# ai4sre/RCAEval

Hardware: AMD Instinct MI355X
Metric: Fisher-z CI tests/sec + PC skeleton wall-time (2000 vars), 1/2/4/8 MI355X (higher is better)
Workload: dtype f64

## Files before the change

include/pcgpu.h:

```cpp
#ifndef PCGPU_H
#define PCGPU_H

#include <stdint.h>

#ifdef __cplusplus
extern "C" {
#endif

#define PCG_OK 0
#define PCG_ERR_INVALID -1
#define PCG_ERR_OOM -2
#define PCG_ERR_HIP -3
#define PCG_ERR_SINGULAR -4
#define PCG_ERR_DOMAIN -5
#define PCG_ERR_RCCL -6
#define PCG_ERR_OVERFLOW -7
#define PCG_ERR_PEER -8

#define PCG_FLAG_FULL_P 0x1
#define PCG_FLAG_RECORD 0x2
#define PCG_FLAG_EXACT_ALL 0x4

#define PCG_MAX_LEVELS 32
#define PCG_MAX_DEPTH 12
// ... 12 lines not shown
    double level_ms[PCG_MAX_LEVELS];
    double kernel_ms[PCG_MAX_LEVELS];
    int32_t levels;
    int32_t error;
    int64_t screened[PCG_MAX_LEVELS];
    int32_t driver;
    int32_t driver_pad;
} pcg_stats;

#define PCG_DRIVER_LEVELS 0
#define PCG_DRIVER_SMALL 1
#define PCG_DRIVER_SMALL_RERUN 2

typedef struct {
    int32_t a, b;
    int32_t d;
    int32_t s[PCG_MAX_DEPTH];
    double p;
} pcg_record;

#define PCG_ABI_VERSION 4
int pcg_abi_info(int64_t *stats_bytes, int64_t *record_bytes, int32_t *version);

int pcg_create(int device, pcg_handle **out);
int pcg_destroy(pcg_handle *h);
const char *pcg_last_error(pcg_handle *h);
int pcg_set_stream(pcg_handle *h, void *hip_stream);
int pcg_set_capacity(pcg_handle *h, int64_t record_capacity, int64_t deferred_capacity);
int pcg_set_record_sample(pcg_handle *h, int64_t modulus, int64_t residue);

#define PCG_TUNE_SMALL 0
#define PCG_TUNE_SMALL_QCAP 1
#define PCG_TUNE_LDS_DEEP 2
#define PCG_TUNE_LDS_SPILL_MIN 3
#define PCG_TUNE_WAVE_LO 4
#define PCG_TUNE_SCREEN_MASK 5
#define PCG_TUNE_NODE_BLOCKS 6
#define PCG_TUNE_EXPORT_INLINE 7
#define PCG_TUNE_NB 8
#define PCG_TUNE_NBW 9
#define PCG_TUNE_HOST_TRACE 10
#define PCG_TUNE_K1_I8 11
#define PCG_TUNE_K1_CRT 12
#define PCG_TUNE_K1_CRT_MINN 13
#define PCG_TUNE_K1_CRT_BITS 14
#define PCG_TUNE_K1_CRT_KS 15
#define PCG_TUNE_K1_I8_KS 16
#define PCG_TUNE_K1_SUPER_ORDER 17
#define PCG_TUNE_L1Z 18
#define PCG_TUNE_K1_CRT_MIX 19
#define PCG_K1_CRT_MIX_FORCED (1ll << 30)
#define PCG_K1_CRT_MIX_FORCE(tA, ksA, ksB) \
    (PCG_K1_CRT_MIX_FORCED | ((int64_t)(tA) << 10) | ((int64_t)(ksA) << 5) | (int64_t)(ksB))
#define PCG_TUNE_COUNT 20
int pcg_set_tuning(pcg_handle *h, int key, int64_t value);
int pcg_get_tuning(pcg_handle *h, int key, int64_t *value);

int pcg_corr(pcg_handle *h, const double *X, int64_t N, int64_t n, int64_t ldx,
             double *C, int64_t ldc);

int pcg_corr_shard_bytes(pcg_handle *h, int64_t n, int64_t N, int world, int64_t *bytes_per_rank);
int pcg_k1_plan_signature(pcg_handle *h, int64_t n, int64_t N, int64_t *signature);
int pcg_k1_crt_plan(pcg_handle *h, int64_t n, int64_t N, int64_t *plan);
int pcg_corr_shard_rows(int64_t n, int world, int64_t *rows_per_rank);
int pcg_corr_shard(pcg_handle *h, const double *X, int64_t N, int64_t n, int64_t ldx, int rank,
                   int world, double *packed);
int pcg_corr_shard_finish(pcg_handle *h, const double *gathered, int64_t N, int64_t n, int world,
                          double *C, int64_t ldc);

int pcg_skeleton(pcg_handle *h, const double *C, int64_t n, int64_t ldc, int64_t N,
                 double alpha, int max_depth, int flags, int8_t *removed_level,
                 pcg_stats *stats);

int pcg_pc_skeleton(pcg_handle *h, const double *X, int64_t N, int64_t n, int64_t ldx, double *C,
                    int64_t ldc, double alpha, int max_depth, int flags, int8_t *removed_level,
                    pcg_stats *stats);

int pcg_degrees(pcg_handle *h, int32_t *deg_host, int64_t capacity);

int pcg_sepset_count(pcg_handle *h, int64_t *count, int32_t *words_per_row);
int pcg_sepset_export(pcg_handle *h, int32_t *xy_host ,
                      uint64_t *bits_host , int64_t count);
int pcg_sepset_export_device(pcg_handle *h, int32_t *xy_dev, uint64_t *bits_dev, int64_t count);
int pcg_set_sepset_buffers(pcg_handle *h, int32_t *xy_dev, uint64_t *bits_dev, int64_t capacity);
int pcg_sepset_target(pcg_handle *h, int32_t *in_caller, int64_t *capacity_needed);

int pcg_record_count(pcg_handle *h, int64_t *count, int64_t *near_alpha_count);
int pcg_record_export(pcg_handle *h, pcg_record *rec_host, int64_t count,
                      pcg_record *near_host, int64_t near_count);

typedef struct {
    const double *X;
    int64_t N, n, ldx;
    double *C;
    int64_t ldc;
    int8_t *removed_level;
    int32_t *sep_xy;
    uint64_t *sep_bits;
} pcg_case;
typedef struct {
    int32_t rc;
    int32_t rc_pad;
    int64_t sep_rows;
    int64_t near_alpha_count;
    pcg_stats stats;
    int32_t deg[PCG_MAX_LEVELS][64];
} pcg_case_result;
// ... 121 lines not shown
```

rcaeval_amd/_lib.py:

```python
from __future__ import annotations

import ctypes
import os

_HERE = os.path.dirname(os.path.abspath(__file__))
LIB_PATH = os.environ.get("PCG_LIB_PATH") or os.path.join(_HERE, "libpcgpu.so")

PCG_OK = 0
PCG_ERR_INVALID = -1
PCG_ERR_OOM = -2
PCG_ERR_HIP = -3
PCG_ERR_SINGULAR = -4
PCG_ERR_DOMAIN = -5
PCG_ERR_RCCL = -6
PCG_ERR_OVERFLOW = -7
PCG_ERR_PEER = -8

PCG_FLAG_FULL_P = 0x1
PCG_FLAG_RECORD = 0x2
PCG_FLAG_EXACT_ALL = 0x4

PCG_MAX_LEVELS = 32
PCG_ABI_VERSION = 4
PCG_RM_STATUS = 64
PCG_MAX_DEPTH = 12
PCG_MAX_LEVEL_DEPTH = 30

PCG_DRIVER_LEVELS = 0
PCG_DRIVER_SMALL = 1
PCG_DRIVER_SMALL_RERUN = 2
DRIVER_NAMES = {PCG_DRIVER_LEVELS: "levels", PCG_DRIVER_SMALL: "small", PCG_DRIVER_SMALL_RERUN: "small_rerun"}

TUNE_KEYS = {
    "SMALL": 0, "SMALL_QCAP": 1, "LDS_DEEP": 2, "LDS_SPILL_MIN": 3, "WAVE_LO": 4, "SCREEN_MASK": 5,
    "NODE_BLOCKS": 6, "EXPORT_INLINE": 7, "NB": 8, "NBW": 9, "HOST_TRACE": 10, "K1_I8": 11, "K1_CRT": 12,
    "K1_CRT_MINN": 13, "K1_CRT_BITS": 14, "K1_CRT_KS": 15, "K1_I8_KS": 16, "K1_SUPER_ORDER": 17,
    "L1Z": 18, "K1_CRT_MIX": 19,
}


def k1_crt_mix_force(tA: int, ksA: int, ksB: int) -> int:
    return (1 << 30) | (int(tA) << 10) | (int(ksA) << 5) | int(ksB)

I64 = ctypes.c_int64
I32 = ctypes.c_int32
P = ctypes.c_void_p
D = ctypes.c_double


class PcgStats(ctypes.Structure):
    _fields_ = [
        ("tests", I64 * PCG_MAX_LEVELS),
        ("calls", I64 * PCG_MAX_LEVELS),
        ("indep", I64 * PCG_MAX_LEVELS),
        ("exact", I64 * PCG_MAX_LEVELS),
        ("near_alpha", I64 * PCG_MAX_LEVELS),
        ("edges_after", I64 * PCG_MAX_LEVELS),
        ("max_degree", I32 * PCG_MAX_LEVELS),
        ("level_ms", D * PCG_MAX_LEVELS),
        ("kernel_ms", D * PCG_MAX_LEVELS),
        ("levels", I32),
        ("error", I32),
        ("screened", I64 * PCG_MAX_LEVELS),
        ("driver", I32),
        ("driver_pad", I32),
    ]

    def as_dict(self) -> dict:
        L = self.levels
        return {
            "levels": L,
            "error": self.error,
            "tests": list(self.tests[:L]),
            "calls": list(self.calls[:L]),
            "indep": list(self.indep[:L]),
            "exact": list(self.exact[:L]),
            "near_alpha": list(self.near_alpha[:L]),
            "edges_after": list(self.edges_after[:L]),
            "max_degree": list(self.max_degree[:L]),
            "level_ms": list(self.level_ms[:L]),
            "kernel_ms": list(self.kernel_ms[:L]),
            "screened": list(self.screened[:L]),
            "driver": DRIVER_NAMES.get(self.driver, str(self.driver)),
        }


class PcgRecord(ctypes.Structure):
    _fields_ = [("a", I32), ("b", I32), ("d", I32), ("s", I32 * PCG_MAX_DEPTH), ("p", D)]


# ... 176 lines not shown
```

rcaeval_amd/csrc/api.hip:

```cpp
#include <hip/hip_runtime.h>

#include <algorithm>
#include <cerrno>
#include <cstdlib>
#include <cstring>

#include "handle.h"

int pcg_fail(pcg_handle *h, int code, const char *fmt, ...) {
    if (h) {
        char buf[1024];
        va_list ap;
        va_start(ap, fmt);
        vsnprintf(buf, sizeof(buf), fmt, ap);
        va_end(ap);
        h->err = buf;
    }
    return code;
}

bool pcg_ensure(pcg_handle *h, DevBuf &b, size_t bytes) {
    if (bytes == 0) bytes = 16;
    if (b.bytes >= bytes) return true;
    if (b.p) {
// ... 25 lines not shown
    ++h->alloc_events;
    if (hipHostMalloc(&b.p, bytes, hipHostMallocMapped) != hipSuccess) {
        b.p = nullptr;
        return false;
    }
    if (hipHostGetDevicePointer(&b.dp, b.p, 0) != hipSuccess) {
        hipHostFree(b.p);
        b.p = b.dp = nullptr;
        return false;
    }
    b.bytes = bytes;
    return true;
}

extern "C" int pcg_abi_info(int64_t *stats_bytes, int64_t *record_bytes, int32_t *version) {
    if (stats_bytes) *stats_bytes = (int64_t)sizeof(pcg_stats);
    if (record_bytes) *record_bytes = (int64_t)sizeof(pcg_record);
    if (version) *version = PCG_ABI_VERSION;
    return PCG_OK;
}

extern "C" int pcg_batch_abi_info(int64_t *case_bytes, int64_t *result_bytes) {
    if (case_bytes) *case_bytes = (int64_t)sizeof(pcg_case);
    if (result_bytes) *result_bytes = (int64_t)sizeof(pcg_case_result);
    return PCG_OK;
}

namespace {
struct TuneSpec {
    const char *env;
    int64_t dflt, lo, hi;
};
const TuneSpec kTune[PCG_TUNE_COUNT] = {
    {"PCG_SMALL", 1, 0, 1},
    {"PCG_SMALL_QCAP", 1024, 1, 1024},
    {"PCG_LDS_DEEP", 20, 12, 20},
    {"PCG_LDS_SPILL_MIN", 10000000, 0, INT64_MAX},
    {"PCG_WAVE_LO", 0, 0, PCG_MAX_LEVEL_DEPTH + 1},
    {"PCG_SCREEN_MASK", -1, -1, 0x1c},
    {"PCG_NODE_BLOCKS", 0x18, 0, 0x1c},
    {"PCG_EXPORT_INLINE", 16384, 0, INT64_MAX},
    {"PCG_NB", 0, 0, 1 << 24},
    {"PCG_NBW", 512, 1, 1 << 24},
    {"PCG_HOST_TRACE", 0, 0, 1},
    {"PCG_K1_I8", 1, 0, 1},
    {"PCG_K1_CRT", 1, 0, 1},
    {"PCG_K1_CRT_MINN", 256, 1, 1 << 24},
    {"PCG_K1_CRT_BITS", 53, 32, 63},
    {"PCG_K1_CRT_KS", 0, 0, 16},
    {"PCG_K1_I8_KS", 0, 0, 256},
    {"PCG_K1_SUPER_ORDER", 1, 0, 1},
    {"PCG_L1Z", 1, 0, 1},
    {"PCG_K1_CRT_MIX", 1, 0, INT32_MAX},
};
}

void pcg_tuning_defaults(int64_t *tune) {
    for (int k = 0; k < PCG_TUNE_COUNT; ++k) {
        int64_t v = kTune[k].dflt;
        if (const char *e = getenv(kTune[k].env)) {
            char *end = nullptr;
            errno = 0;
            const long long p = strtoll(e, &end, 0);
            if (end == e || *end != '\0' || errno == ERANGE || p < kTune[k].lo || p > kTune[k].hi)
                fprintf(stderr, "pcgpu: ignoring %s=%s (not an integer in [%lld, %lld]); using %lld\n", kTune[k].env, e,
                        (long long)kTune[k].lo, (long long)kTune[k].hi, (long long)kTune[k].dflt);
            else
                v = p;
        }
        tune[k] = v;
    }
}

extern "C" int pcg_set_tuning(pcg_handle *h, int key, int64_t value) {
    if (!h || key < 0 || key >= PCG_TUNE_COUNT || value < kTune[key].lo || value > kTune[key].hi)
        return pcg_fail(h, PCG_ERR_INVALID, "pcg_set_tuning: key %d value %lld", key, (long long)value);
    h->tune[key] = value;
    return PCG_OK;
}

extern "C" int pcg_get_tuning(pcg_handle *h, int key, int64_t *value) {
    if (!h || !value || key < 0 || key >= PCG_TUNE_COUNT)
        return pcg_fail(h, PCG_ERR_INVALID, "pcg_get_tuning: key %d", key);
    *value = h->tune[key];
    return PCG_OK;
}

extern "C" int pcg_create(int device, pcg_handle **out) {
    if (!out) return PCG_ERR_INVALID;
    *out = nullptr;
    int ndev = 0;
    if (hipGetDeviceCount(&ndev) != hipSuccess || ndev <= 0) return PCG_ERR_HIP;
    if (device < 0 || device >= ndev) return PCG_ERR_INVALID;
    if (hipSetDevice(device) != hipSuccess) return PCG_ERR_HIP;
    pcg_handle *h = new pcg_handle();
    h->device = device;
    pcg_tuning_defaults(h->tune);
    if (hipStreamCreateWithFlags(&h->stream, hipStreamNonBlocking) != hipSuccess) {
        delete h;
        return PCG_ERR_HIP;
    }
    h->own_stream = true;
    for (auto &e : h->ev)
        if (hipEventCreate(&e) != hipSuccess) {
            delete h;
            return PCG_ERR_HIP;
        }
    *out = h;
    return PCG_OK;
}

extern "C" int pcg_destroy(pcg_handle *h) {
    if (!h) return PCG_OK;
    hipSetDevice(h->device);
    if (h->stream) hipStreamSynchronize(h->stream);
    pcg_comm_release(h);
    if (h->xs) hipStreamSynchronize(h->xs);
    DevBuf *bufs[] = {&h->adj, &h->deg, &h->off2[0], &h->off2[1], &h->nbr2[0], &h->nbr2[1], &h->rm, &h->ug2[0],
                      &h->ug2[1], &h->exp_ctr, &h->cpre, &h->binom, &h->ctr,
                      &h->deferred, &h->screenq, &h->records, &h->nearbuf, &h->exportbuf, &h->export_xy, &h->diag,
                      &h->colmean, &h->pr_scratch, &h->batch_scratch, &h->chisq_scratch, &h->cblk, &h->lmk, &h->ibo,
                      &h->k1_digits, &h->small_sum, &h->batch_up, &h->batch_sum, &h->batch_near,
                      &h->granger_scratch, &h->granger_work, &h->lingam_w, &h->lingam_z, &h->lingam_d,
                      &h->lingam_small, &h->pcmci_e, &h->pcmci_r, &h->pcmci_small, &h->pcmci_work,
                      &h->fges_e, &h->fges_r, &h->fges_small, &h->fges_list, &h->fges_work, &h->scaler_up,
                      &h->cmlp_scratch, &h->cmlp_best};
    for (DevBuf *b : bufs)
        if (b->p) hipFree(b->p);
    PinBuf *pins[] = {&h->ctr_pin, &h->deg_pin, &h->off_pin, &h->cpre_pin, &h->status_pin, &h->small_pin,
                      &h->batch_up_pin, &h->batch_sum_pin};
    for (PinBuf *b : pins)
        if (b->p) hipHostFree(b->p);
    if (h->summary) hipHostFree(h->summary);
    for (auto &e : h->ev)
        if (e) hipEventDestroy(e);
    for (auto &e : h->lev)
        if (e) hipEventDestroy(e);
    for (auto &pr : h->rev)
        for (auto &e : pr)
            if (e) hipEventDestroy(e);
    if (h->ev_join) hipEventDestroy(h->ev_join);
    if (h->ev_fork) hipEventDestroy(h->ev_fork);
    if (h->tail) hipHostFree(h->tail);
    if (h->aux) hipStreamDestroy(h->aux);
    if (h->xs) hipStreamDestroy(h->xs);
    if (h->ev_xready) hipEventDestroy(h->ev_xready);
    for (auto &e : h->ev_xdone)
        if (e) hipEventDestroy(e);
    if (h->own_stream && h->stream) hipStreamDestroy(h->stream);
    delete h;
// ... 36 lines not shown
```

rcaeval_amd/csrc/corr.hip:

```cpp
#include <hip/hip_runtime.h>

#include <algorithm>
#include <cmath>
#include <cstring>
#include <vector>

#include "handle.h"

namespace {

typedef double d4 __attribute__((ext_vector_type(4)));

#ifndef PCG_K1_TILE
#define PCG_K1_TILE 64
#endif
#ifndef PCG_K1_XCD
#define PCG_K1_XCD 1
#endif
#ifndef PCG_K1_KS
#define PCG_K1_KS 0
#endif
constexpr int TILE = PCG_K1_TILE;
constexpr int WT = TILE / 32;
constexpr int RS = 256 / TILE;
// ... 342 lines not shown
    _Pragma("unroll") for (int q = 0; q < K1_DIG; ++q)                                 \
        reinterpret_cast<v4i *>(&st[(buf_)][0][0])[q * 256 + tid] = pre[q];
    if (tb0 < tb1) {
        K1_LOAD(tb0);
        K1_STORE(0);
    }
    __syncthreads();
    for (int tb = tb0; tb < tb1; ++tb) {
        const int buf = (tb - tb0) & 1;
        if (tb + 1 < tb1) { K1_LOAD(tb + 1); }
        v4i bq[K1_DIG];
#pragma unroll
        for (int q = 0; q < K1_DIG; ++q)
            bq[q] = *reinterpret_cast<const v4i *>(&st[buf][K1_DIG + q][hh * 1024 + (wc + r) * 16]);
#pragma unroll
        for (int p = 0; p < K1_DIG; ++p) {
            const v4i ap = *reinterpret_cast<const v4i *>(&st[buf][p][hh * 1024 + (wr + r) * 16]);
#pragma unroll
            for (int q = 0; q < K1_DIG - p; ++q)
                acc[p + q] = __builtin_amdgcn_mfma_i32_32x32x32_i8(ap, bq[q], acc[p + q], 0, 0, 0);
        }
        if (tb + 1 < tb1) { K1_STORE(buf ^ 1); }
        __syncthreads();
    }
#undef K1_LOAD
#undef K1_STORE
    const int j = bj * 64 + wc + r;
    const int ej = j < n ? expo[j] : 0;
#pragma unroll
    for (int k = 0; k < 16; ++k) {
        const int i = bi * 64 + wr + (k & 3) + 8 * (k >> 2) + 4 * hh;
        if (i >= n || j >= n) continue;
        const int ei = expo[i];
        double v = 0.0;
        if (ei == K1_NONFINITE || ej == K1_NONFINITE) {
            v = NAN;
        } else {
#pragma unroll
            for (int l = K1_LEVELS - 1; l >= 0; --l)
                v += ldexp((double)acc[l][k], ei + ej - 7 * (l + 2));
        }
        if (pbi >= 0) {
            G[((int64_t)pbi * 64 + (i - bi * 64)) * ldg + j] = v;
        } else if (bi != bj || i <= j) {
            G[(int64_t)i * ldg + j] = v;
        }
    }
}

constexpr int CRT_KMAX = 24;
constexpr int CRT_L = 6;
constexpr int CRT_T = 256;
constexpr int CRT_KB = 4;
#ifndef PCG_CRT_PR
#define PCG_CRT_PR 8
#endif
constexpr int CRT_PR = PCG_CRT_PR;
#ifndef PCG_CRT_KP
#define PCG_CRT_KP 1
#endif
constexpr int CRT_KP = PCG_CRT_KP;
constexpr int CRT_PL = CRT_PR - 2 * CRT_KP;
static_assert(CRT_PR * 16384 <= 160 * 1024 && CRT_PL >= CRT_KP && CRT_PL % CRT_KP == 0, "CRT LDS ring");
constexpr int CRT_MAXKB = 4095;
constexpr int CRT_UNIT = CRT_T * CRT_T;
static const int kCrtModuli[CRT_KMAX] = {256, 255, 253, 251, 247, 241, 239, 233, 229, 227, 223, 217,
                                         211, 199, 197, 193, 191, 181, 179, 173, 167, 163, 157, 151};

struct CrtTab {
    int k, b, L;
    int m[CRT_KMAX];
    int y[CRT_KMAX];
    float finv[CRT_KMAX];
    double dinv[CRT_KMAX];
    uint32_t wlo[CRT_KMAX], whi[CRT_KMAX];
    uint32_t cneg[CRT_KMAX];
    uint32_t Mi[CRT_KMAX][2 * CRT_L];
    uint32_t M[2 * CRT_L];
};

struct CrtSplit {
    int tA, ksA, kbA, ksB, kbB;
    int64_t nA;
};

__device__ __forceinline__ void crt_tile_units(const CrtSplit &sp, int ntiles, int t, int &ks, int64_t &base,
                                               int64_t &ustride) {
    const bool inA = t < sp.tA;
    ks = inA ? sp.ksA : sp.ksB;
    base = inA ? (int64_t)t : sp.nA + (t - sp.tA);
    ustride = (int64_t)(inA ? sp.tA : ntiles - sp.tA) * CRT_UNIT;
}

template <int L>
struct CrtAcc {
    uint32_t l[2 * L];
    float fs;
};

template <int L>
__device__ __forceinline__ void crt_acc_init(CrtAcc<L> &a) {
#pragma unroll
    for (int l = 0; l < 2 * L; ++l) a.l[l] = 0;
    a.fs = 0.0f;
}

template <int L>
__device__ __forceinline__ void crt_acc_add(CrtAcc<L> &a, uint32_t z, int mi, const CrtTab &tab) {
    a.fs = fmaf((float)z, tab.finv[mi], a.fs);
#pragma unroll
    for (int l = 0; l < 2 * L; ++l) a.l[l] = __umul24(z, tab.Mi[mi][l]) + a.l[l];
}

template <int L>
__device__ __forceinline__ double crt_value(const CrtAcc<L> &a, const CrtTab &tab, int ei, int ej) {
    const int32_t qq = (int32_t)floorf(a.fs + 0.5f);
// ... 77 lines not shown
    const double *xp = X + t0 * ldx + j;
#pragma unroll
    for (int i = 0; i < 16; ++i) {
        const double v = (live && t0 + i < N) ? xp[(int64_t)i * ldx] - mu : 0.0;
        const double y = ldexp(fabs(v), tab.b - e);
        const uint32_t h = (uint32_t)(y * 0x1p-32);
        const uint32_t l = (uint32_t)(y - (double)h * 0x1p32);
        const bool neg = v < 0.0;
        lo[i] = neg ? 0u - l : l;
        hi[i] = neg ? B - h - (l != 0u) : B + h;
    }
    const int64_t plane = (int64_t)CBp * TB * 2048;
    int8_t *dst = R + ((int64_t)cb * TB + tb) * 2048 + half * 1024 + c * 16;
    auto pack4 = [](uint32_t b0, uint32_t b1, uint32_t b2, uint32_t b3) {
        const uint32_t w01 = __builtin_amdgcn_perm(b1, b0, 0x0c0c0400u);
        const uint32_t w23 = __builtin_amdgcn_perm(b3, b2, 0x0c0c0400u);
        return __builtin_amdgcn_perm(w23, w01, 0x05040100u);
    };
    for (int mi = m0; mi < m1; ++mi) {
        v4i pk;
        const int m = tab.m[mi];
        if (m == 256) {
#pragma unroll
            for (int q = 0; q < 4; ++q) pk[q] = (int)pack4(lo[4 * q], lo[4 * q + 1], lo[4 * q + 2], lo[4 * q + 3]);
        } else {
            const f2 fi = {tab.finv[mi], tab.finv[mi]};
            const f2 nm = {-(float)m, -(float)m};
            const f2 mg = {12582912.0f, 12582912.0f};
            const uint32_t wl = tab.wlo[mi], wh = tab.whi[mi], cn = tab.cneg[mi];
#pragma unroll
            for (int q = 0; q < 4; ++q) {
                uint32_t bb[4];
#pragma unroll
                for (int u = 0; u < 4; u += 2) {
                    const int i = 4 * q + u;
                    const float x0 = (float)(int)__builtin_amdgcn_udot4(
                        lo[i], wl, __builtin_amdgcn_udot4(hi[i], wh, cn, false), false);
                    const float x1 = (float)(int)__builtin_amdgcn_udot4(
                        lo[i + 1], wl, __builtin_amdgcn_udot4(hi[i + 1], wh, cn, false), false);
                    const f2 x = {x0, x1};
                    const f2 qv = __builtin_elementwise_fma(x, fi, mg) - mg;
                    const f2 rv = __builtin_elementwise_fma(qv, nm, x) + mg;
                    const float r0 = rv.x, r1 = rv.y;
                    bb[u] = __float_as_uint(r0);
                    bb[u + 1] = __float_as_uint(r1);
                }
                pk[q] = (int)pack4(bb[0], bb[1], bb[2], bb[3]);
            }
        }
        *reinterpret_cast<v4i *>(dst + mi * plane) = pk;
    }
}

__global__ __launch_bounds__(512, 1) void k_xtx_crt(const int8_t *R, int TB, int64_t plane, int T, int ntiles,
                                                  CrtSplit sp, CrtTab tab, int64_t u0, int64_t nu, int64_t nuA,
                                                  unsigned gA, uint8_t *out) {
    extern __shared__ __attribute__((aligned(16))) unsigned char smem[];
    int64_t lin;
    {
        const bool blkA = blockIdx.x < gA;
        const unsigned b = blkA ? blockIdx.x : blockIdx.x - gA;
        const int64_t per = (blkA ? gA : gridDim.x - gA) / 8;
        lin = (b % 8) * per + b / 8;
        if (lin >= (blkA ? nuA : nu - nuA)) return;
        if (!blkA) lin += nuA;
    }
    const int64_t u = u0 + lin;
    const bool inA = u < sp.nA;
    const int64_t v = inA ? u : u - sp.nA;
    const int tc = inA ? sp.tA : ntiles - sp.tA;
    const int ks = inA ? sp.ksA : sp.ksB, kb = inA ? sp.kbA : sp.kbB;
    const int t = (int)(v % tc) + (inA ? 0 : sp.tA);
    const int64_t sm = v / tc;
    const int mi = (int)(sm / ks), slab = (int)(sm % ks);
    int bi, bj;
    tile_of(t, T, bi, bj);
    const int tb0 = slab * kb, tb1 = min(TB, tb0 + kb);
    const int tid = threadIdx.x, lane = tid & 63, w = tid >> 6;
    const int r = lane & 31, hh = lane >> 5;
    const int wr = w >> 2, wc = w & 3;

    v16i acc[4][2];
#pragma unroll
    for (int a = 0; a < 4; ++a)
#pragma unroll
        for (int b = 0; b < 2; ++b)
#pragma unroll
            for (int q = 0; q < 16; ++q) acc[a][b][q] = 0;

    const int8_t *Rm = R + (int64_t)mi * plane;
    const int8_t *srcA = Rm + (int64_t)(bi * 4 + (tid >> 7)) * TB * 2048 + (tid & 127) * 16;
    const int8_t *srcB = Rm + (int64_t)(bj * 4 + (tid >> 7)) * TB * 2048 + (tid & 127) * 16;
    const int nkb = tb1 - tb0;
    auto stage = [&](int g) {
        const int64_t tb = tb0 + min(g, nkb - 1);
        unsigned char *dst = smem + (g % CRT_PR) * 16384 + w * 1024;
        __builtin_amdgcn_global_load_lds((const __attribute__((address_space(1))) void *)(srcA + tb * 2048),
                                         (__attribute__((address_space(3))) void *)dst, 16, 0, 0);
        __builtin_amdgcn_global_load_lds((const __attribute__((address_space(1))) void *)(srcB + tb * 2048),
                                         (__attribute__((address_space(3))) void *)(dst + 8192), 16, 0, 0);
    };
    const unsigned char *fa0 = smem + (2 * wr * 2048 + hh * 1024 + r * 16);
    const unsigned char *fb0 = smem + (8192 + wc * 2048 + hh * 1024 + r * 16);
    v4i af[2][CRT_KP][4], bf[2][CRT_KP][2];
    auto frag = [&](int g, int sl) {
#pragma unroll
        for (int kk = 0; kk < CRT_KP; ++kk) {
            const int off = ((g + kk) % CRT_PR) * 16384;
#pragma unroll
            for (int a = 0; a < 4; ++a)
                af[sl][kk][a] = *reinterpret_cast<const v4i *>(fa0 + off + (a >> 1) * 2048 + (a & 1) * 512);
#pragma unroll
            for (int b = 0; b < 2; ++b) bf[sl][kk][b] = *reinterpret_cast<const v4i *>(fb0 + off + b * 512);
        }
    };
#pragma unroll
    for (int g = 0; g < CRT_PL; ++g) stage(g);
    asm volatile("s_waitcnt vmcnt(%0)" ::"n"(2 * (CRT_PL - CRT_KP)) : "memory");
    __builtin_amdgcn_s_barrier();
    frag(0, 0);
    for (int p = 0; p < nkb; p += 2 * CRT_KP) {
#pragma unroll
        for (int h2 = 0; h2 < 2; ++h2) {
            const int q = p + h2 * CRT_KP;
            if (q < nkb) {
#pragma unroll
                for (int kk = 0; kk < CRT_KP; ++kk) stage(q + CRT_PL + kk);
                asm volatile("s_waitcnt vmcnt(%0)" ::"n"(2 * (CRT_PL - CRT_KP)) : "memory");
                __builtin_amdgcn_s_barrier();
                const bool nxt = q + CRT_KP < nkb;
                if (nxt) frag(q + CRT_KP, h2 ^ 1);
#pragma unroll
                for (int kk = 0; kk < CRT_KP; ++kk) {
                    if (kk > 0 && q + kk >= nkb) break;
#pragma unroll
                    for (int a = 0; a < 4; ++a)
#pragma unroll
                        for (int b = 0; b < 2; ++b)
                            acc[a][b] = __builtin_amdgcn_mfma_i32_32x32x32_i8(af[h2][kk][a], bf[h2][kk][b], acc[a][b],
                                                                              0, 0, 0);
                }
                if (nxt) {
#pragma unroll
                    for (int u = 0; u < 6 * CRT_KP; ++u) {
                        __builtin_amdgcn_sched_group_barrier(0x008, 1, 0);
                        __builtin_amdgcn_sched_group_barrier(0x100, 1, 0);
                    }
                    __builtin_amdgcn_sched_group_barrier(0x008, 2 * CRT_KP, 0);
                }
            }
        }
    }
    asm volatile("s_waitcnt vmcnt(0)" ::: "memory");
    const int m = tab.m[mi];
    const float fm = (float)m, finv = tab.finv[mi];
    const int c16 = (int)((tab.wlo[mi] >> 16) & 0xffu);
    uint8_t *o = out + lin * CRT_UNIT + (int64_t)w * 8192 + lane * 16;
#pragma unroll
    for (int a = 0; a < 4; ++a)
#pragma unroll
        for (int b = 0; b < 2; ++b) {
            v4i pk = {0, 0, 0, 0};
#pragma unroll
            for (int q = 0; q < 16; ++q) {
                const int v = acc[a][b][q];
                uint32_t rr;
                if (m == 256) {
                    rr = (uint32_t)v & 255u;
                } else {
                    const int t = __mul24(v >> 16, c16) + (v & 0xffff);
                    const float tf = (float)t;
                    int x = (int)fmaf(-rintf(tf * finv), fm, tf);
                    x += x < 0 ? m : 0;
                    x -= x >= m ? m : 0;
                    rr = (uint32_t)x;
                }
                pk[q >> 2] |= (int)(rr << (8 * (q & 3)));
            }
            *reinterpret_cast<v4i *>(o + (a * 2 + b) * 1024) = pk;
        }
}

__device__ __forceinline__ int crt_unit_offset(int li, int lj) {
    const int wr = li >> 7, a = (li >> 5) & 3, rr = li & 31;
    const int hh = (rr >> 2) & 1, q = (rr & 3) | ((rr >> 3) << 2);
    const int wc = lj >> 6, b = (lj >> 5) & 1, r = lj & 31;
    return ((((wr * 4 + wc) * 4 + a) * 2 + b) * 64 + r + 32 * hh) * 16 + q;
}

template <int L>
__global__ __launch_bounds__(256) void k_crt_diag(const uint8_t *Rs, int T, int ntiles, CrtSplit sp, CrtTab tab,
                                                 const int *expo, int n, double scale, double *sd) {
    const int i = blockIdx.x * blockDim.x + threadIdx.x;
    if (i >= n) return;
    const int bi = blockIdx.x;
    const int t = bi * T - bi * (bi - 1) / 2;
    const int ei = expo[i];
    if (ei == K1_NONFINITE) {
        sd[i] = NAN;
        return;
    }
    const int k = tab.k;
    int ks;
    int64_t ubase, ustride;
    crt_tile_units(sp, ntiles, t, ks, ubase, ustride);
    const uint8_t *src = Rs + ubase * CRT_UNIT + crt_unit_offset(i % CRT_T, i % CRT_T);
    uint32_t sv[CRT_KMAX];
#pragma unroll
    for (int mi = 0; mi < CRT_KMAX; ++mi) sv[mi] = 0;
    for (int s = 0; s < ks; ++s) {
        uint32_t b[CRT_KMAX];
#pragma unroll
        for (int mi = 0; mi < CRT_KMAX; ++mi) b[mi] = src[((int64_t)min(mi, k - 1) * ks + s) * ustride];
#pragma unroll
        for (int mi = 0; mi < CRT_KMAX; ++mi) sv[mi] += b[mi];
    }
    CrtAcc<L> acc;
    crt_acc_init(acc);
#pragma unroll
    for (int mi = 0; mi < CRT_KMAX; ++mi)
        if (mi < k) crt_acc_add(acc, crt_mod(__umul24(sv[mi], (uint32_t)tab.y[mi]), tab.m[mi], tab.finv[mi]), mi, tab);
    sd[i] = sqrt(crt_value(acc, tab, ei, ei) * scale);
}

template <int L>
__global__ __launch_bounds__(256) void k_crt_finish(const uint8_t *Rs, int T, int ntiles, CrtSplit sp, CrtTab tab,
                                                   const int *expo, int n, const double *sd, double scale, double *C,
                                                   int64_t ldc) {
    const int64_t gid = (int64_t)blockIdx.x * blockDim.x + threadIdx.x;
    const int rem = (int)((gid >> 2) & 4095), g = (int)(gid & 3);
    const int t = (int)(blockIdx.x >> 6);
    if (t >= ntiles) return;
    int bi, bj;
    tile_of(t, T, bi, bj);
// ... 255 lines not shown
        t.wlo[i] = wl;
        t.whi[i] = wh;
        uint64_t pb = 1;
        for (int s2 = 0; s2 < b; ++s2) pb = (pb * 2) % m;
        t.cneg[i] = 0u - (uint32_t)pb;
    }
    p.T = (n + CRT_T - 1) / CRT_T;
    p.ntiles = p.T * (p.T + 1) / 2;
    p.CBp = p.T * 4;
    p.TB = (int)((N + 63) / 64 * 2);
    int best = 1;
    double best_cost = 1e300;
    const int force = (int)tune[PCG_TUNE_K1_CRT_KS];
    for (int ks = 1; ks <= 16; ++ks) {
        int kbk = (p.TB + ks - 1) / ks;
        kbk = (kbk + CRT_KB - 1) / CRT_KB * CRT_KB;
        const int kse = (p.TB + kbk - 1) / kbk;
        if (kse != ks || kbk > CRT_MAXKB) continue;
        const int64_t U = (int64_t)p.ntiles * k * ks;
        const double cost = force > 0 ? (double)std::abs(ks - force)
                                      : (double)((U + 255) / 256) * kbk * 0.3 + (double)U * 0.026;
        if (cost < best_cost) {
            best_cost = cost;
            best = ks;
        }
    }
    {
        int kbk = (p.TB + best - 1) / best;
        kbk = (kbk + CRT_KB - 1) / CRT_KB * CRT_KB;
        if (kbk > CRT_MAXKB) return false;
        p.kb = kbk;
        p.ks = (p.TB + kbk - 1) / kbk;
    }
    p.units = (int64_t)p.ntiles * k * p.ks;
    p.sp = CrtSplit{p.ntiles, p.ks, p.kb, p.ks, p.kb, p.units};
    if (mixed) crt_plan_mix(tune[PCG_TUNE_K1_CRT_MIX], p);
    return true;
}

int crt_residues(pcg_handle *h, const CrtPlan &p, const double *X, int64_t N, int nn, int64_t ldx, const double *mean,
                 const int *expo, int m0, int m1, hipStream_t st, const int8_t **R) {
    const size_t bytes = (size_t)p.tab.k * p.CBp * p.TB * 2048;
    if (!pcg_ensure(h, h->k1_digits, bytes)) return pcg_fail(h, PCG_ERR_OOM, "K1 residue planes (%zu bytes)", bytes);
    hipLaunchKernelGGL(k_residues, dim3((unsigned)p.CBp, (unsigned)(p.TB / 2)), dim3(256), 0, st, X, N, nn, ldx, mean,
                       expo, p.CBp, p.TB, p.tab, m0, m1, (int8_t *)h->k1_digits.p);
    *R = (const int8_t *)h->k1_digits.p;
    return PCG_OK;
}

void crt_gemm(pcg_handle *h, const CrtPlan &p, const int8_t *R, int64_t u0, int64_t nu, uint8_t *out) {
    if (nu <= 0) return;
    const int64_t plane = (int64_t)p.CBp * p.TB * 2048;
    const int64_t nuA = std::min(nu, std::max<int64_t>(p.sp.nA - u0, 0));
    const unsigned gA = (unsigned)((nuA + 7) / 8 * 8), gB = (unsigned)((nu - nuA + 7) / 8 * 8);
    hipLaunchKernelGGL(k_xtx_crt, dim3(gA + gB), dim3(512), CRT_PR * 16384, h->stream, R, p.TB, plane, p.T,
                       p.ntiles, p.sp, p.tab, u0, nu, nuA, gA, out);
}

void crt_finish(pcg_handle *h, const CrtPlan &p, const uint8_t *Rs, const int *expo, int nn, int64_t N, double *sd,
                double *C, int64_t ldc) {
    const double scale = 1.0 / (double)(N - 1);
    const int64_t threads = (int64_t)p.ntiles * 16384;
#define CRT_LAUNCH(L_)                                                                                       \
    do {                                                                                                     \
        hipLaunchKernelGGL((k_crt_diag<L_>), dim3((unsigned)((nn + CRT_T - 1) / CRT_T)), dim3(CRT_T), 0,      \
                           h->stream, Rs, p.T, p.ntiles, p.sp, p.tab, expo, nn, scale, sd);                   \
        hipLaunchKernelGGL((k_crt_finish<L_>), dim3((unsigned)((threads + 255) / 256)), dim3(256), 0,         \
                           h->stream, Rs, p.T, p.ntiles, p.sp, p.tab, expo, nn, (const double *)sd, scale, C, \
                           ldc);                                                                              \
    } while (0)
    if (p.tab.L <= 4) { CRT_LAUNCH(4); }
    else if (p.tab.L == 5) { CRT_LAUNCH(5); }
    else { CRT_LAUNCH(6); }
#undef CRT_LAUNCH
}

int k1_digits(pcg_handle *h, const double *X, int64_t N, int nn, int64_t ldx, const double *mean, const int *expo,
              int *CB, int *TB, const int8_t **Dg) {
    *CB = (nn + 63) / 64;
    *TB = (int)((N + 63) / 64 * 2);
    const size_t bytes = (size_t)K1_DIG * *CB * *TB * 2048;
    if (!pcg_ensure(h, h->k1_digits, bytes)) return pcg_fail(h, PCG_ERR_OOM, "K1 digit planes (%zu bytes)", bytes);
    hipLaunchKernelGGL(k_digits, dim3((unsigned)*CB, (unsigned)(*TB / 2)), dim3(256), 0, h->stream, X, N, nn, ldx,
                       mean, expo, *CB, *TB, (int8_t *)h->k1_digits.p);
    *Dg = (const int8_t *)h->k1_digits.p;
    return PCG_OK;
}

constexpr int NT = 64;
__device__ __forceinline__ double slab_diag_sd(const double *G, int64_t ldg, int64_t slab_stride, int ks, int i,
                                               double scale) {
    double v = 0.0;
    for (int s = 0; s < ks; ++s) v += G[(int64_t)s * slab_stride + (int64_t)i * ldg + i];
    return sqrt(v * scale);
}

__global__ __launch_bounds__(256) void k_normalize_tiles(const double *G, int64_t ldg, int64_t slab_stride, int ks,
                                                         double *C, int64_t ldc, int n, double scale) {
    __shared__ double t[NT][NT + 1];
    __shared__ double sdr[NT], sdc[NT];
    const int T = (n + NT - 1) / NT;
    int bi = 0, bj = 0;
    {
        int r = blockIdx.x;
        while (r >= T - bi) { r -= T - bi; ++bi; }
        bj = bi + r;
    }
    const int i0 = bi * NT, j0 = bj * NT;
    const int c = threadIdx.x & 63, r4 = threadIdx.x >> 6;
// ... 546 lines not shown
```

rcaeval_amd/csrc/handle.h:

```cpp
#pragma once
#include <hip/hip_runtime.h>

#include <cstdarg>
#include <cstdint>
#include <cstdio>
#include <string>
#include <vector>
#include <chrono>

#include "pcgpu.h"

struct DevBuf {
    void *p = nullptr;
    size_t bytes = 0;
};

struct PinBuf {
    void *p = nullptr;
    void *dp = nullptr;
    size_t bytes = 0;
};

struct DevCounters {
    unsigned long long tests;
    unsigned long long indep;
    unsigned long long deferred;
    unsigned long long exact;
    unsigned long long records;
    unsigned long long near_alpha;
    unsigned long long exported;
    unsigned long long error;
    unsigned long long screened;
    unsigned long long t_run0, t_run1;
};

struct LevelSummary {
    DevCounters ctr;
    uint8_t status[8];
    int32_t ug_clean;
    long long img_total;
    unsigned long long stamp;
    unsigned long long seq;
};

struct ScreenEntry {
    int32_t x, y;
    int32_t s[4];
};

struct DeferredEntry {
    int32_t x, y;
    int32_t s[PCG_MAX_DEPTH];
};

inline double pcg_now_us() {
    return std::chrono::duration<double, std::micro>(std::chrono::steady_clock::now().time_since_epoch()).count();
}
#define PCG_HT(h, label) \
    do { if ((h)->htrace_on) (h)->htrace.emplace_back((label), pcg_now_us()); } while (0)

struct pcg_handle {
    int device = 0;
    int64_t tune[PCG_TUNE_COUNT] = {};
    hipStream_t stream = nullptr;
    bool own_stream = false;
    std::string err;
    hipEvent_t ev[4] = {nullptr, nullptr, nullptr, nullptr};
    hipEvent_t lev[2] = {};
    bool lev_on = false;

    DevBuf screenq;
    DevBuf adj, deg, rm, cpre, binom, ctr, deferred, records, nearbuf, exportbuf, export_xy, diag, colmean,
        pr_scratch, batch_scratch, chisq_scratch;
    DevBuf granger_scratch, granger_work;
    DevBuf lingam_w, lingam_z, lingam_d, lingam_small;
    DevBuf pcmci_e, pcmci_r, pcmci_small, pcmci_work;
    int64_t pcmci_shape[3] = {0, 0, 0};
    bool pcmci_ok = false;
    DevBuf fges_e, fges_r, fges_small, fges_list, fges_work;
    int64_t fges_shape[2] = {0, 0};
    bool fges_ok = false;
    DevBuf scaler_up;
    bool scaler_lds_set = false;
    DevBuf cmlp_scratch, cmlp_best;
    DevBuf k1_digits;
    int64_t k1_stamp[4] = {0, 0, 0, 0};
    bool k1_stamp_ok = false;
    DevBuf off2[2], nbr2[2], ug2[2];
    int cb = 0;
    bool ug_clean2[2] = {false, false};
    unsigned long long ug_pend_seq = 0;
    int ug_pend_set = 0;
    hipStream_t xs = nullptr;
    hipEvent_t ev_xready = nullptr, ev_xdone[2] = {nullptr, nullptr};
    bool xpending[2] = {false, false};
    bool xany = false;
    bool xinl = false;
    DevBuf exp_ctr;
    PinBuf ctr_pin, deg_pin, off_pin, cpre_pin, status_pin;
    DevBuf small_sum;
    PinBuf small_pin;
    DevBuf batch_up, batch_sum, batch_near;
    PinBuf batch_up_pin, batch_sum_pin;
    std::vector<std::vector<pcg_record>> batch_near_h;
    std::vector<uint64_t> binom_h;
    uint8_t *rm_ext = nullptr;
    const uint8_t *banned = nullptr;
    int64_t rm_ext_bytes = 0;
    int64_t rec_cap = 0, def_cap = 1 << 20, near_cap = 1 << 16, scr_cap = 1 << 20;
    int64_t rec_mod = 0, rec_res = 0;
    int64_t export_cap = 0;
    int64_t export_rows = 0;
    int32_t *usr_xy = nullptr;
    uint64_t *usr_bits = nullptr;
    int64_t usr_cap = 0;
// ... 153 lines not shown
```

Baseline: 1451 billion.

## Make CRT int8 GEMM kernel persistent with cross-unit prefetch pipeline

Converts k_xtx_crt from one block per output unit to a persistent grid capped near the CU count. Each block loops over units, and the LDS staging ring keeps prefetching the next unit's K-slabs while the current unit's epilogue runs. Unit metadata is computed in scalar registers. This targets per-block launch and pipeline fill/drain overhead, at the cost of more complex vmcnt bookkeeping and possible load imbalance on the tail. A new tuning key, an optional timestamp probe, and a CU-count query at handle creation are also added.

```diff
diff --git a/include/pcgpu.h b/include/pcgpu.h
--- a/include/pcgpu.h
+++ b/include/pcgpu.h
@@ -88,7 +88,8 @@
 #define PCG_K1_CRT_MIX_FORCED (1ll << 30)
 #define PCG_K1_CRT_MIX_FORCE(tA, ksA, ksB) \
     (PCG_K1_CRT_MIX_FORCED | ((int64_t)(tA) << 10) | ((int64_t)(ksA) << 5) | (int64_t)(ksB))
-#define PCG_TUNE_COUNT 20
+#define PCG_TUNE_K1_CRT_GRID 20
+#define PCG_TUNE_COUNT 21
 int pcg_set_tuning(pcg_handle *h, int key, int64_t value);
 int pcg_get_tuning(pcg_handle *h, int key, int64_t *value);
 
diff --git a/rcaeval_amd/_lib.py b/rcaeval_amd/_lib.py
--- a/rcaeval_amd/_lib.py
+++ b/rcaeval_amd/_lib.py
@@ -35,7 +35,7 @@
     "SMALL": 0, "SMALL_QCAP": 1, "LDS_DEEP": 2, "LDS_SPILL_MIN": 3, "WAVE_LO": 4, "SCREEN_MASK": 5,
     "NODE_BLOCKS": 6, "EXPORT_INLINE": 7, "NB": 8, "NBW": 9, "HOST_TRACE": 10, "K1_I8": 11, "K1_CRT": 12,
     "K1_CRT_MINN": 13, "K1_CRT_BITS": 14, "K1_CRT_KS": 15, "K1_I8_KS": 16, "K1_SUPER_ORDER": 17,
-    "L1Z": 18, "K1_CRT_MIX": 19,
+    "L1Z": 18, "K1_CRT_MIX": 19, "K1_CRT_GRID": 20,
 }
 
 
diff --git a/rcaeval_amd/csrc/api.hip b/rcaeval_amd/csrc/api.hip
--- a/rcaeval_amd/csrc/api.hip
+++ b/rcaeval_amd/csrc/api.hip
@@ -101,6 +101,7 @@
     {"PCG_K1_SUPER_ORDER", 1, 0, 1},
     {"PCG_L1Z", 1, 0, 1},
     {"PCG_K1_CRT_MIX", 1, 0, INT32_MAX},
+    {"PCG_K1_CRT_GRID", 0, 0, INT32_MAX},
 };
 }
 
@@ -145,6 +146,10 @@
     pcg_handle *h = new pcg_handle();
     h->device = device;
     pcg_tuning_defaults(h->tune);
+    if (hipDeviceGetAttribute(&h->cus, hipDeviceAttributeMultiprocessorCount, device) != hipSuccess || h->cus <= 0) {
+        delete h;
+        return PCG_ERR_HIP;
+    }
     if (hipStreamCreateWithFlags(&h->stream, hipStreamNonBlocking) != hipSuccess) {
         delete h;
         return PCG_ERR_HIP;
diff --git a/rcaeval_amd/csrc/corr.hip b/rcaeval_amd/csrc/corr.hip
--- a/rcaeval_amd/csrc/corr.hip
+++ b/rcaeval_amd/csrc/corr.hip
@@ -418,16 +418,9 @@
 constexpr int CRT_L = 6;
 constexpr int CRT_T = 256;
 constexpr int CRT_KB = 4;
-#ifndef PCG_CRT_PR
-#define PCG_CRT_PR 8
-#endif
-constexpr int CRT_PR = PCG_CRT_PR;
-#ifndef PCG_CRT_KP
-#define PCG_CRT_KP 1
-#endif
-constexpr int CRT_KP = PCG_CRT_KP;
-constexpr int CRT_PL = CRT_PR - 2 * CRT_KP;
-static_assert(CRT_PR * 16384 <= 160 * 1024 && CRT_PL >= CRT_KP && CRT_PL % CRT_KP == 0, "CRT LDS ring");
+constexpr int CRT_PR = 8;
+constexpr int CRT_PL = CRT_PR - 1;
+static_assert(CRT_PR * 16384 <= 160 * 1024 && CRT_KB % 2 == 0, "CRT LDS ring");
 constexpr int CRT_MAXKB = 4095;
 constexpr int CRT_UNIT = CRT_T * CRT_T;
 static const int kCrtModuli[CRT_KMAX] = {256, 255, 253, 251, 247, 241, 239, 233, 229, 227, 223, 217,
@@ -611,19 +604,27 @@
     }
 }
 
-__global__ __launch_bounds__(512, 1) void k_xtx_crt(const int8_t *R, int TB, int64_t plane, int T, int ntiles,
-                                                  CrtSplit sp, CrtTab tab, int64_t u0, int64_t nu, int64_t nuA,
-                                                  unsigned gA, uint8_t *out) {
-    extern __shared__ __attribute__((aligned(16))) unsigned char smem[];
+struct CrtUnitAt {
     int64_t lin;
-    {
-        const bool blkA = blockIdx.x < gA;
-        const unsigned b = blkA ? blockIdx.x : blockIdx.x - gA;
-        const int64_t per = (blkA ? gA : gridDim.x - gA) / 8;
-        lin = (b % 8) * per + b / 8;
-        if (lin >= (blkA ? nuA : nu - nuA)) return;
-        if (!blkA) lin += nuA;
-    }
+    int64_t offA, offB;
+    int mi, nkb;
+};
+
+__device__ __forceinline__ int crt_sgpr(int x) { return __builtin_amdgcn_readfirstlane(x); }
+__device__ __forceinline__ int64_t crt_sgpr(int64_t x) {
+    return (int64_t)(((uint64_t)(uint32_t)crt_sgpr((int)((uint64_t)x >> 32)) << 32) | (uint32_t)crt_sgpr((int)x));
+}
+__device__ __forceinline__ CrtUnitAt crt_unit_at(int64_t vb, unsigned gA, unsigned gT, int64_t u0, int64_t nu,
+                                                 int64_t nuA, const CrtSplit &sp, int T, int ntiles, int TB,
+                                                 int64_t plane) {
+    CrtUnitAt c;
+    const bool blkA = vb < gA;
+    const uint64_t b = (uint64_t)(blkA ? vb : vb - gA);
+    const int64_t per = (blkA ? gA : gT - gA) / 8;
+    int64_t lin = (int64_t)(b % 8) * per + (int64_t)(b / 8);
+    const bool real = lin < (blkA ? nuA : nu - nuA);
+    if (!real) lin = 0;
+    if (!blkA) lin += nuA;
     const int64_t u = u0 + lin;
     const bool inA = u < sp.nA;
     const int64_t v = inA ? u : u - sp.nA;
@@ -635,9 +636,41 @@
     int bi, bj;
     tile_of(t, T, bi, bj);
     const int tb0 = slab * kb, tb1 = min(TB, tb0 + kb);
+    const int64_t base = (int64_t)mi * plane + (int64_t)tb0 * 2048;
+    c.lin = crt_sgpr(lin);
+    c.offA = crt_sgpr(base + (int64_t)bi * 4 * TB * 2048);
+    c.offB = crt_sgpr(base + (int64_t)bj * 4 * TB * 2048);
+    c.mi = crt_sgpr(mi);
+    c.nkb = crt_sgpr(real ? tb1 - tb0 : 0);
+    return c;
+}
+
+#ifdef PCG_CRT_STAMP
+__device__ unsigned long long g_crt_stamp[4];
+#define CRT_STAMP(x) const uint64_t x = __builtin_amdgcn_s_memtime()
+#else
+#define CRT_STAMP(x)
+#endif
+
+__global__ __launch_bounds__(512, 1) void k_xtx_crt(const int8_t *R, int TB, int64_t plane, int T, int ntiles,
+                                                  CrtSplit sp, CrtTab tab, int64_t u0, int64_t nu, int64_t nuA,
+                                                  unsigned gA, unsigned gT, uint8_t *out) {
+    extern __shared__ __attribute__((aligned(16))) unsigned char smem[];
     const int tid = threadIdx.x, lane = tid & 63, w = tid >> 6;
     const int r = lane & 31, hh = lane >> 5;
     const int wr = w >> 2, wc = w & 3;
+    const int64_t G = gridDim.x;
+    auto next_unit = [&](int64_t &vb) __attribute__((always_inline)) {
+        CrtUnitAt c{};
+        for (; vb < gT; vb += G) {
+            c = crt_unit_at(vb, gA, gT, u0, nu, nuA, sp, T, ntiles, TB, plane);
+            if (c.nkb) break;
+        }
+        return c;
+    };
+    int64_t cvb = blockIdx.x;
+    CrtUnitAt cu = next_unit(cvb);
+    if (cvb >= gT) return;
 
     v16i acc[4][2];
 #pragma unroll
@@ -647,98 +680,145 @@
 #pragma unroll
             for (int q = 0; q < 16; ++q) acc[a][b][q] = 0;
 
-    const int8_t *Rm = R + (int64_t)mi * plane;
-    const int8_t *srcA = Rm + (int64_t)(bi * 4 + (tid >> 7)) * TB * 2048 + (tid & 127) * 16;
-    const int8_t *srcB = Rm + (int64_t)(bj * 4 + (tid >> 7)) * TB * 2048 + (tid & 127) * 16;
-    const int nkb = tb1 - tb0;
-    auto stage = [&](int g) {
-        const int64_t tb = tb0 + min(g, nkb - 1);
-        unsigned char *dst = smem + (g % CRT_PR) * 16384 + w * 1024;
-        __builtin_amdgcn_global_load_lds((const __attribute__((address_space(1))) void *)(srcA + tb * 2048),
+    const int8_t *Rt = R + (int64_t)(tid >> 7) * TB * 2048 + (tid & 127) * 16;
+    int64_t svb = cvb, s_offA = cu.offA, s_offB = cu.offB, s_step = 2048;
+    int s_rem = cu.nkb, sslot = 0;
+    auto stager_next = [&]() __attribute__((always_inline)) {
+        if (s_rem) return;
+        svb += G;
+        const CrtUnitAt c = next_unit(svb);
+        const bool more = svb < gT;
+        s_offA = more ? c.offA : s_offA - 2048;
+        s_offB = more ? c.offB : s_offB - 2048;
+        s_step = more ? 2048 : 0;
+        s_rem = more ? c.nkb : INT32_MAX;
+    };
+    auto stage = [&]() __attribute__((always_inline)) {
+        unsigned char *dst = smem + sslot * 16384 + w * 1024;
+        __builtin_amdgcn_global_load_lds((const __attribute__((address_space(1))) void *)(Rt + s_offA),
                                          (__attribute__((address_space(3))) void *)dst, 16, 0, 0);
-        __builtin_amdgcn_global_load_lds((const __attribute__((address_space(1))) void *)(srcB + tb * 2048),
+        __builtin_amdgcn_global_load_lds((const __attribute__((address_space(1))) void *)(Rt + s_offB),
                                          (__attribute__((address_space(3))) void *)(dst + 8192), 16, 0, 0);
+        sslot = (sslot + 1) % CRT_PR;
+        s_offA += s_step;
+        s_offB += s_step;
+        --s_rem;
     };
     const unsigned char *fa0 = smem + (2 * wr * 2048 + hh * 1024 + r * 16);
     const unsigned char *fb0 = smem + (8192 + wc * 2048 + hh * 1024 + r * 16);
-    v4i af[2][CRT_KP][4], bf[2][CRT_KP][2];
-    auto frag = [&](int g, int sl) {
-#pragma unroll
-        for (int kk = 0; kk < CRT_KP; ++kk) {
-            const int off = ((g + kk) % CRT_PR) * 16384;
-#pragma unroll
-            for (int a = 0; a < 4; ++a)
-                af[sl][kk][a] = *reinterpret_cast<const v4i *>(fa0 + off + (a >> 1) * 2048 + (a & 1) * 512);
-#pragma unroll
-            for (int b = 0; b < 2; ++b) bf[sl][kk][b] = *reinterpret_cast<const v4i *>(fb0 + off + b * 512);
-        }
+    v4i af[2][4], bf[2][2];
+    int fslot = 0;
+    auto frag = [&](int sl) __attribute__((always_inline)) {
+        const int off = fslot * 16384;
+#pragma unroll
+        for (int a = 0; a < 4; ++a)
+            af[sl][a] = *reinterpret_cast<const v4i *>(fa0 + off + (a >> 1) * 2048 + (a & 1) * 512);
+#pragma unroll
+        for (int b = 0; b < 2; ++b) bf[sl][b] = *reinterpret_cast<const v4i *>(fb0 + off + b * 512);
+        fslot = (fslot + 1) % CRT_PR;
     };
-#pragma unroll
-    for (int g = 0; g < CRT_PL; ++g) stage(g);
-    asm volatile("s_waitcnt vmcnt(%0)" ::"n"(2 * (CRT_PL - CRT_KP)) : "memory");
+    auto region = [&](int h2) __attribute__((always_inline)) {
+        frag(h2 ^ 1);
+        stage();
+#pragma unroll
+        for (int a = 0; a < 4; ++a)
+#pragma unroll
+            for (int b = 0; b < 2; ++b)
+                acc[a][b] = __builtin_amdgcn_mfma_i32_32x32x32_i8(af[h2][a], bf[h2][b], acc[a][b], 0, 0, 0);
+#pragma unroll
+        for (int u = 0; u < 3; ++u) {
+            __builtin_amdgcn_sched_group_barrier(0x008, 1, 0);
+            __builtin_amdgcn_sched_group_barrier(0x100, 2, 0);
+        }
+        __builtin_amdgcn_sched_group_barrier(0x008, 1, 0);
+#pragma unroll
+        for (int u = 0; u < 2; ++u) {
+            __builtin_amdgcn_sched_group_barrier(0x008, 1, 0);
+            __builtin_amdgcn_sched_group_barrier(0x020, 1, 0);
+        }
+        __builtin_amdgcn_sched_group_barrier(0x008, 2, 0);
+    };
+#pragma unroll 1
+    for (int g = 0; g < CRT_PL; ++g) {
+        stager_next();
+        stage();
+    }
+    asm volatile("s_waitcnt vmcnt(%0)" ::"n"(2 * (CRT_PL - 1)) : "memory");
     __builtin_amdgcn_s_barrier();
-    frag(0, 0);
-    for (int p = 0; p < nkb; p += 2 * CRT_KP) {
-#pragma unroll
-        for (int h2 = 0; h2 < 2; ++h2) {
-            const int q = p + h2 * CRT_KP;
-            if (q < nkb) {
-#pragma unroll
-                for (int kk = 0; kk < CRT_KP; ++kk) stage(q + CRT_PL + kk);
-                asm volatile("s_waitcnt vmcnt(%0)" ::"n"(2 * (CRT_PL - CRT_KP)) : "memory");
+    frag(0);
+#ifdef PCG_CRT_STAMP
+    uint64_t st_b = 0, st_c = 0, st_n = 0;
+    const uint64_t st_t0 = __builtin_amdgcn_s_memtime();
+#endif
+    int young = 0;
+    for (;;) {
+        for (int j = 0; j < cu.nkb; j += 2) {
+#pragma unroll
+            for (int h2 = 0; h2 < 2; ++h2) {
+                stager_next();
+                CRT_STAMP(t0);
+                if (young > 0) {
+                    asm volatile("s_waitcnt vmcnt(%0)" ::"n"(2 * (CRT_PL - 2) + 8) : "memory");
+                    --young;
+                } else {
+                    asm volatile("s_waitcnt vmcnt(%0)" ::"n"(2 * (CRT_PL - 2)) : "memory");
+                }
                 __builtin_amdgcn_s_barrier();
-                const bool nxt = q + CRT_KP < nkb;
-                if (nxt) frag(q + CRT_KP, h2 ^ 1);
-#pragma unroll
-                for (int kk = 0; kk < CRT_KP; ++kk) {
-                    if (kk > 0 && q + kk >= nkb) break;
-#pragma unroll
-                    for (int a = 0; a < 4; ++a)
-#pragma unroll
-                        for (int b = 0; b < 2; ++b)
-                            acc[a][b] = __builtin_amdgcn_mfma_i32_32x32x32_i8(af[h2][kk][a], bf[h2][kk][b], acc[a][b],
-                                                                              0, 0, 0);
+                CRT_STAMP(t1);
+                region(h2);
+#ifdef PCG_CRT_STAMP
+                __builtin_amdgcn_sched_barrier(0);
+                CRT_STAMP(t2);
+                st_b += t1 - t0;
+                st_c += t2 - t1;
+                ++st_n;
+#endif
+            }
+        }
+        const int mi = cu.mi, m = tab.m[mi];
+        const float fm = (float)m, finv = tab.finv[mi];
+        const int c16 = (int)((tab.wlo[mi] >> 16) & 0xffu);
+        uint8_t *o = out + cu.lin * CRT_UNIT + (int64_t)w * 8192 + lane * 16;
+#pragma unroll
+        for (int a = 0; a < 4; ++a)
+#pragma unroll
+            for (int b = 0; b < 2; ++b) {
+                v4i pk = {0, 0, 0, 0};
+#pragma unroll
+                for (int q = 0; q < 16; ++q) {
+                    const int v = acc[a][b][q];
+                    acc[a][b][q] = 0;
+                    uint32_t rr;
+                    if (m == 256) {
+                        rr = (uint32_t)v & 255u;
+                    } else {
+                        const int t = __mul24(v >> 16, c16) + (v & 0xffff);
+                        const float tf = (float)t;
+                        int x = (int)fmaf(-rintf(tf * finv), fm, tf);
+                        x += x < 0 ? m : 0;
+                        x -= x >= m ? m : 0;
+                        rr = (uint32_t)x;
+                    }
+                    pk[q >> 2] |= (int)(rr << (8 * (q & 3)));
                 }
-                if (nxt) {
-#pragma unroll
-                    for (int u = 0; u < 6 * CRT_KP; ++u) {
-                        __builtin_amdgcn_sched_group_barrier(0x008, 1, 0);
-                        __builtin_amdgcn_sched_group_barrier(0x100, 1, 0);
-                    }
-                    __builtin_amdgcn_sched_group_barrier(0x008, 2 * CRT_KP, 0);
-                }
+                *reinterpret_cast<v4i *>(o + (a * 2 + b) * 1024) = pk;
             }
-        }
-    }
+        young = CRT_PL - 1;
+        cvb += G;
+        cu = next_unit(cvb);
+        if (cvb >= gT) break;
+    }
+#ifdef PCG_CRT_STAMP
+    if (lane == 0) {
+        atomicAdd(&g_crt_stamp[0], st_b);
+        atomicAdd(&g_crt_stamp[1], st_c);
+        atomicAdd(&g_crt_stamp[2], st_n);
+        atomicAdd(&g_crt_stamp[3], __builtin_amdgcn_s_memtime() - st_t0);
+    }
+#endif
     asm volatile("s_waitcnt vmcnt(0)" ::: "memory");
-    const int m = tab.m[mi];
-    const float fm = (float)m, finv = tab.finv[mi];
-    const int c16 = (int)((tab.wlo[mi] >> 16) & 0xffu);
-    uint8_t *o = out + lin * CRT_UNIT + (int64_t)w * 8192 + lane * 16;
-#pragma unroll
-    for (int a = 0; a < 4; ++a)
-#pragma unroll
-        for (int b = 0; b < 2; ++b) {
-            v4i pk = {0, 0, 0, 0};
-#pragma unroll
-            for (int q = 0; q < 16; ++q) {
-                const int v = acc[a][b][q];
-                uint32_t rr;
-                if (m == 256) {
-                    rr = (uint32_t)v & 255u;
-                } else {
-                    const int t = __mul24(v >> 16, c16) + (v & 0xffff);
-                    const float tf = (float)t;
-                    int x = (int)fmaf(-rintf(tf * finv), fm, tf);
-                    x += x < 0 ? m : 0;
-                    x -= x >= m ? m : 0;
-                    rr = (uint32_t)x;
-                }
-                pk[q >> 2] |= (int)(rr << (8 * (q & 3)));
-            }
-            *reinterpret_cast<v4i *>(o + (a * 2 + b) * 1024) = pk;
-        }
-}
+}
+#undef CRT_STAMP
 
 __device__ __forceinline__ int crt_unit_offset(int li, int lj) {
     const int wr = li >> 7, a = (li >> 5) & 3, rr = li & 31;
@@ -1100,9 +1180,22 @@
     if (nu <= 0) return;
     const int64_t plane = (int64_t)p.CBp * p.TB * 2048;
     const int64_t nuA = std::min(nu, std::max<int64_t>(p.sp.nA - u0, 0));
-    const unsigned gA = (unsigned)((nuA + 7) / 8 * 8), gB = (unsigned)((nu - nuA + 7) / 8 * 8);
-    hipLaunchKernelGGL(k_xtx_crt, dim3(gA + gB), dim3(512), CRT_PR * 16384, h->stream, R, p.TB, plane, p.T,
-                       p.ntiles, p.sp, p.tab, u0, nu, nuA, gA, out);
+    const unsigned gA = (unsigned)((nuA + 7) / 8 * 8), gB = (unsigned)((nu - nuA + 7) / 8 * 8), gT = gA + gB;
+    const int64_t cap = h->tune[PCG_TUNE_K1_CRT_GRID] > 0 ? h->tune[PCG_TUNE_K1_CRT_GRID]
+                                                          : std::max(8, h->cus / 8 * 8);
+    const unsigned G = (unsigned)std::min<int64_t>(gT, cap);
+    hipLaunchKernelGGL(k_xtx_crt, dim3(G), dim3(512), CRT_PR * 16384, h->stream, R, p.TB, plane, p.T, p.ntiles, p.sp,
+                       p.tab, u0, nu, nuA, gA, gT, out);
+#ifdef PCG_CRT_STAMP
+    {
+        unsigned long long st[4], z[4] = {0, 0, 0, 0};
+        hipStreamSynchronize(h->stream);
+        hipMemcpyFromSymbol(st, HIP_SYMBOL(g_crt_stamp), sizeof(st));
+        hipMemcpyToSymbol(HIP_SYMBOL(g_crt_stamp), z, sizeof(z));
+        fprintf(stderr, "[crt stamp] phases %llu: wait+barrier %.1f, mfma cluster %.1f, loop total %.1f cycles per phase\n",
+                st[2], (double)st[0] / st[2], (double)st[1] / st[2], (double)st[3] / st[2]);
+    }
+#endif
 }
 
 void crt_finish(pcg_handle *h, const CrtPlan &p, const uint8_t *Rs, const int *expo, int nn, int64_t N, double *sd,
diff --git a/rcaeval_amd/csrc/handle.h b/rcaeval_amd/csrc/handle.h
--- a/rcaeval_amd/csrc/handle.h
+++ b/rcaeval_amd/csrc/handle.h
@@ -61,6 +61,7 @@
 
 struct pcg_handle {
     int device = 0;
+    int cus = 0;
     int64_t tune[PCG_TUNE_COUNT] = {};
     hipStream_t stream = nullptr;
     bool own_stream = false;
```

Result: no change. 1450 billion (-0.1%).
